# soldasim/BOSS.jl

Measured on AMD Instinct MI355X. Metric: gp_posterior_updates_per_sec (+ acq_evals_per_sec), N=4096 d=8 fp64, higher is better.
Workload: dtype f64; 1 GPU; d=8 synthetic blackbox, GaussianProcess(Matern52) surrogate, N=4096 fp64 posterior update + ExpectedImprovement over 8192 candidates per GPU (BASELINE.json configs[1]+[2]); N=4096, d=8, M_per_gpu=8192, kernel=matern52, parallelism=single GPU: no exchange

## Files before the change

### boss.jl_amd/api.py

```python
from __future__ import annotations

import ctypes as C
import os
from typing import Optional, Sequence

import numpy as np

_HERE = os.path.dirname(os.path.abspath(__file__))
LIB_PATH = os.environ.get("BOSS_LIB_PATH") or os.path.join(_HERE, "libbosship.so")

BOSS_OK, BOSS_E_INVALID, BOSS_E_NO_DEVICE, BOSS_E_NOT_PD, BOSS_E_NEG_VAR, BOSS_E_NOT_FITTED, BOSS_E_ALLOC = range(7)
KERNELS = {"matern32": 0, "matern52": 1, "sqexp": 2}
FIT_NO_SYNC = 1

_c_dp = C.POINTER(C.c_double)
_c_ucp = C.POINTER(C.c_ubyte)

SIGNATURES = {
    "boss_version": (C.c_char_p, []),
    "boss_last_error": (C.c_char_p, []),
    "boss_device_count": (C.c_int, [C.POINTER(C.c_int)]),
    "boss_set_stream": (C.c_int, [C.c_int, C.c_void_p]),
    "boss_device_sync": (C.c_int, [C.c_int]),
    "boss_gp_create": (C.c_int, [C.c_int, C.c_int, C.c_int, C.c_int, _c_dp, _c_dp, _c_ucp, C.POINTER(C.c_void_p)]),
# ... 2216 lines not shown

def _fallbacks(device: int = 0):
    lib = load_library()
    fn = lib.boss_debug_fallbacks
    fn.restype = C.c_int
    fn.argtypes = [C.c_int, C.POINTER(C.c_long), C.POINTER(C.c_int)]
    n, off = C.c_long(0), C.c_int(0)
    _check(fn(device, C.byref(n), C.byref(off)))
    return n.value, off.value


def _set_launches(device: int = 0):
    lib = load_library()
    fn = lib.boss_debug_set_launches
    fn.restype = C.c_int
    fn.argtypes = [C.c_int, C.POINTER(C.c_long), C.POINTER(C.c_long)]
    a, b = C.c_long(0), C.c_long(0)
    fn(device, C.byref(a), C.byref(b))
    return a.value, b.value


def _set_grad_launches(device: int = 0):
    lib = load_library()
    fn = lib.boss_debug_set_grad_launches
    fn.restype = C.c_int
    fn.argtypes = [C.c_int, C.POINTER(C.c_long)]
    a = C.c_long(0)
    fn(device, C.byref(a))
    return a.value


def _acq_path(device: int = 0):
    fn = load_library().boss_debug_acq_path
    fn.restype = C.c_int
    fn.argtypes = [C.c_int, C.POINTER(C.c_int)]
    out = (C.c_int * 5)()
    _check(fn(device, out))
    return tuple(out)


def _acq_prune_set(device: int = 0, min_tiles: int = -1, K: int = -1, s: int = -1, cap: int = -1, slack: Optional[float] = None):
    lib = load_library()
    fn = lib.boss_debug_acq_prune_set
    fn.restype = C.c_int
    fn.argtypes = [C.c_int] * 5
    _check(fn(device, int(min_tiles), int(K), int(s), int(cap)))
    if slack is not None:
        fs = lib.boss_debug_acq_prune_slack
        fs.restype = C.c_int
        fs.argtypes = [C.c_int, C.c_double]
        _check(fs(device, float(slack)))


def _acq_prune_bounds(M: int, device: int = 0):
    fn = load_library().boss_debug_acq_prune_bounds
    fn.restype = C.c_int
    fn.argtypes = [C.c_int, C.c_int, C.c_void_p, C.c_void_p, C.c_void_p]
    mua, vs, ub = np.zeros(M), np.zeros(M), np.zeros(M)
    _check(fn(device, int(M), mua.ctypes.data, vs.ctypes.data, ub.ctypes.data))
    return mua, vs, ub


def _acq_counters(g: GP):
    fn = load_library().boss_debug_acq_counters
    fn.restype = C.c_int
    fn.argtypes = [C.c_void_p, C.POINTER(C.c_long)]
    out = (C.c_long * 4)()
    _check(fn(g._h, out))
    return tuple(out)
```

### boss.jl_amd/csrc/bosship.hip

```cpp
#include "../../include/bosship.h"

#include <hip/hip_runtime.h>

#include <algorithm>
#include <cmath>
#include <cstdint>
#include <cstdio>
#include <cstdlib>
#include <atomic>
#include <chrono>
#include <cstring>
#include <functional>
#include <limits>
#include <map>
#include <mutex>
#include <string>
#include <thread>
#include <vector>

#include "gp_kernels.hpp"
#include "potrf.hpp"
#include "chain.hpp"
#include "small_calls.hpp"
#include "rider.hpp"
// ... 47 lines not shown
        (void)hipDeviceSynchronize();
    }
    return e;
}

constexpr size_t MULTI_RES_OFF = 384;
constexpr size_t FEW_RES_OFF = 400;

struct Workspace {
    void* p = nullptr;
    size_t bytes = 0;
};

struct Ctx {
    int device = -1;
    int logical = -1;
    hipStream_t own_stream = nullptr;
    hipStream_t stream = nullptr;
    hipStream_t side_stream = nullptr;
    std::vector<hipEvent_t> ev_panel, ev_rest;
    hipEvent_t ev_fork = nullptr, ev_up = nullptr;
    unsigned long long* sig_panel = nullptr;
    unsigned long long* sig_panel_host = nullptr;
    unsigned long long sig_seq = 0;
    hipStream_t chain_stream = nullptr, strip_stream = nullptr;
    unsigned long long chain_seq = 0, crit_seq = 0, up_seq = 0;
    int n_cus = 256;
    bool chain_ok = false;
    bool test_drop_chain = false;
    unsigned long long acq_seq = 0;
    unsigned long long few_seq = 0;
    std::mutex slab_mtx;
    void* slab_cache = nullptr;
    size_t slab_cache_bytes = 0;
    void* hostblk_cache = nullptr;
    size_t hostblk_cache_bytes = 0;
    unsigned long long* few_done = nullptr;
    unsigned long long few_done_cnt = 0;
    long set_launches = 0, set_pre_launches = 0;
    long set_grad_launches = 0;
    bool lookahead = true;
    bool prof_on = false;
    std::map<std::string, std::vector<std::pair<hipEvent_t, hipEvent_t>>> prof;
    std::vector<hipEvent_t> ev_pool;
    Workspace vscratch, csc, pred, acq, batchA, batchX, batchMisc, craw, lgA, lgB, lgC, few, setdesc, setmom, gsetdesc, nlatjobs, mceps, meanws, warpws, prunews;
    static constexpr int LLG_BANKS = 4;
    Workspace lgbank[LLG_BANKS - 1][3];
    hipStream_t llg_stream[LLG_BANKS - 1] = {nullptr, nullptr, nullptr};
    hipEvent_t llg_join[LLG_BANKS - 1] = {nullptr, nullptr, nullptr};
    void* pinned = nullptr;
    int prune_last[5] = {0, 0, 0, 0, 0};
    long prune_launches = 0;
    int prune_M = 0;
    struct TrailTab {
        TrailWork* dev = nullptr;
        std::vector<TrailWork> host;
        std::vector<int> off;
    };
    TrailTab trail[65];
    std::mutex mtx;
};

static void chain_quiesce(Ctx* c) {
    if (c->chain_stream) (void)hipStreamSynchronize(c->chain_stream);
    if (c->strip_stream) (void)hipStreamSynchronize(c->strip_stream);
}

static std::mutex g_ctx_mtx;
static std::map<int, Ctx*> g_ctx;

static bool release_cached_slabs() {
    int dev = -1;
    if (hipGetDevice(&dev) != hipSuccess) return false;
    std::vector<void*> blocks;
    {
        std::lock_guard<std::mutex> lk(g_ctx_mtx);
        for (auto& kv : g_ctx) {
            Ctx* c = kv.second;
            if (c->device != dev) continue;
            std::lock_guard<std::mutex> sl(c->slab_mtx);
            if (c->slab_cache) blocks.push_back(c->slab_cache);
            c->slab_cache = nullptr;
            c->slab_cache_bytes = 0;
        }
    }
    for (void* b : blocks) (void)hipFree(b);
    return !blocks.empty();
}
extern "C" int boss_debug_fail_next_alloc(int n) {
    g_fail_allocs.store(n > 0 ? n : 0);
    return BOSS_OK;
}
extern "C" int boss_debug_slab_cache_bytes(int device, size_t* bytes_out) {
    std::lock_guard<std::mutex> lk(g_ctx_mtx);
    auto it = g_ctx.find(device);
    if (bytes_out) *bytes_out = 0;
    if (it != g_ctx.end() && bytes_out) {
        std::lock_guard<std::mutex> sl(it->second->slab_mtx);
        *bytes_out = it->second->slab_cache_bytes;
    }
    return BOSS_OK;
}

extern "C" int boss_debug_set_launches(int device, long* all_out, long* pre_out) {
    std::lock_guard<std::mutex> lk(g_ctx_mtx);
    auto it = g_ctx.find(device);
    if (all_out) *all_out = it != g_ctx.end() ? it->second->set_launches : 0;
    if (pre_out) *pre_out = it != g_ctx.end() ? it->second->set_pre_launches : 0;
    return BOSS_OK;
}

extern "C" int boss_debug_set_grad_launches(int device, long* out) {
    std::lock_guard<std::mutex> lk(g_ctx_mtx);
    auto it = g_ctx.find(device);
    if (out) *out = it != g_ctx.end() ? it->second->set_grad_launches : 0;
    return BOSS_OK;
}

static void ctx_destroy(Ctx* c) {
    if (!c) return;
    if (c->own_stream) (void)hipStreamDestroy(c->own_stream);
    if (c->side_stream) (void)hipStreamDestroy(c->side_stream);
    if (c->chain_stream) (void)hipStreamDestroy(c->chain_stream);
    if (c->strip_stream) (void)hipStreamDestroy(c->strip_stream);
    if (c->ev_fork) (void)hipEventDestroy(c->ev_fork);
    if (c->sig_panel && !c->sig_panel_host) (void)hipFree(c->sig_panel);
    if (c->few_done) (void)hipFree(c->few_done);
    for (auto& t : c->trail)
        if (t.dev) (void)hipFree(t.dev);
    if (c->slab_cache) (void)hipFree(c->slab_cache);
    if (c->hostblk_cache) (void)hipHostFree(c->hostblk_cache);
    if (c->ev_up) (void)hipEventDestroy(c->ev_up);
    for (int i = 0; i < Ctx::LLG_BANKS - 1; ++i) {
        if (c->llg_stream[i]) (void)hipStreamDestroy(c->llg_stream[i]);
        if (c->llg_join[i]) (void)hipEventDestroy(c->llg_join[i]);
    }
    if (c->pinned) (void)hipHostFree(c->pinned);
    delete c;
}

static int ctx_init(Ctx* c) {
    {
        int least = 0, greatest = 0;
        (void)hipDeviceGetStreamPriorityRange(&least, &greatest);
        static const int cu_mask = getenv("BOSS_CU_MASK") ? atoi(getenv("BOSS_CU_MASK")) : 0;
        if (cu_mask) {
            hipDeviceProp_t prop;
            HIPCHK(hipGetDeviceProperties(&prop, c->device));
            const int ncu = prop.multiProcessorCount, words = (ncu + 31) / 32;
            auto make = [&](hipStream_t* st, int lo, int hi) {
                std::vector<uint32_t> m(words, 0u);
                for (int b = lo; b < hi && b < ncu; ++b) m[b / 32] |= 1u << (b % 32);
                return hipExtStreamCreateWithCUMask(st, (uint32_t)words, m.data());
            };
            HIPCHK(make(&c->chain_stream, 0, 16));
            HIPCHK(make(&c->strip_stream, 16, 32));
            HIPCHK(make(&c->own_stream, 32, ncu));
            HIPCHK(make(&c->side_stream, cu_mask >= 2 ? 40 : 32, cu_mask >= 2 ? ncu : ncu - 8));
            c->stream = c->own_stream;
            std::fprintf(stderr, "[bosship] BOSS_CU_MASK=%d: chain on CU bits 0-15, strips on 16-31, main stream on 32-%d, side stream %d-%d\n",
                         cu_mask, ncu - 1, cu_mask >= 2 ? 40 : 32, (cu_mask >= 2 ? ncu : ncu - 8) - 1);
        } else {
        HIPCHK(hipStreamCreateWithPriority(&c->own_stream, hipStreamNonBlocking, greatest));
        c->stream = c->own_stream;
        HIPCHK(hipStreamCreateWithPriority(&c->side_stream, hipStreamNonBlocking, least));
        HIPCHK(hipStreamCreateWithPriority(&c->chain_stream, hipStreamNonBlocking, greatest));
        HIPCHK(hipStreamCreateWithPriority(&c->strip_stream, hipStreamNonBlocking, greatest));
        }
    }
    HIPCHK(hipEventCreateWithFlags(&c->ev_fork, hipEventDisableTiming));
    HIPCHK(hipEventCreateWithFlags(&c->ev_up, hipEventDisableTiming));
    for (int i = 0; i < Ctx::LLG_BANKS - 1; ++i) {
        HIPCHK(hipStreamCreateWithFlags(&c->llg_stream[i], hipStreamNonBlocking));
        HIPCHK(hipEventCreateWithFlags(&c->llg_join[i], hipEventDisableTiming));
    }
    c->lookahead = !(getenv("BOSS_NO_LOOKAHEAD") && atoi(getenv("BOSS_NO_LOOKAHEAD")));
    {
        auto set_nonzero = [](const char* name) {
            const char* v = getenv(name);
            return v && *v && std::strcmp(v, "0") != 0;
        };
        static const bool gate_off = set_nonzero("BOSS_NO_GATE") || set_nonzero("ROCPROF_COUNTER_COLLECTION") || getenv("ROCPROF_COUNTERS") ||
                                     getenv("ROCPROF_COUNTER_GROUPS") || set_nonzero("ROCPROF_ADVANCED_THREAD_TRACE") ||
                                     getenv("ROCPROF_ATT_PARAM_SERIALIZE_ALL") || getenv("ROCP_METRICS") || set_nonzero("AMD_SERIALIZE_KERNEL");
        if (!gate_off) {
            if (set_nonzero("BOSS_DEBUG_WATCH")) {
                unsigned long long* hp = nullptr;
                HIPCHK(hipHostMalloc((void**)&hp, SIG_WORDS * sizeof(unsigned long long), hipHostMallocMapped));
                std::memset(hp, 0, SIG_WORDS * sizeof(unsigned long long));
                HIPCHK(hipHostGetDevicePointer((void**)&c->sig_panel, hp, 0));
                c->sig_panel_host = hp;
#ifdef BOSS_DEBUG_WATCH_BUILD
                HIPCHK(hipMemcpyToSymbol(HIP_SYMBOL(boss::g_dbg), &c->sig_panel, sizeof(void*)));
#endif
                std::thread([hp]() {
                    unsigned long long last[SIG_WORDS] = {0};
                    for (;;) {
                        std::this_thread::sleep_for(std::chrono::milliseconds(500));
                        unsigned long long now[SIG_WORDS];
                        for (int i = 0; i < SIG_WORDS; ++i) now[i] = ((volatile unsigned long long*)hp)[i];
                        if (std::memcmp(now, last, sizeof now) == 0) continue;
                        std::memcpy(last, now, sizeof now);
                        std::fprintf(stderr, "[bosship watch] up %llu wdone %llu panel %llu crit %llu | gate %llu near %llu bulk %llu | strips",
                                     now[SIGW_UP], now[SIGW_WDONE], now[SIGW_PANEL], now[SIGW_CRIT], now[SIGW_GATE], now[SIGW_NEAR], now[SIGW_BULK]);
                        for (int q = 0; q < 8; ++q) std::fprintf(stderr, " %llu", now[SIGW_PROG + SIGW_PROG_STRIDE * q]);
                        std::fprintf(stderr, " | give-ups: first %llu n %llu last %llu; waits ended by mark %llu, by clock %llu", now[SIGW_DBG], now[SIGW_DBG + 1],
                                     now[SIGW_DBG + 2], now[SIGW_DBG + 4], now[SIGW_DBG + 5]);
                        std::fprintf(stderr, "\n");
                    }
                }).detach();
            } else {
                HIPCHK(hipMalloc((void**)&c->sig_panel, SIG_WORDS * sizeof(unsigned long long)));
                HIPCHK(hipMemset(c->sig_panel, 0, SIG_WORDS * sizeof(unsigned long long)));
            }
        }
        c->chain_ok = !gate_off && !set_nonzero("BOSS_NO_CHAIN") && !set_nonzero("HIP_LAUNCH_BLOCKING");
        c->test_drop_chain = set_nonzero("BOSS_TEST_DROP_CHAIN");
        if (c->chain_ok) {
            int* okw = nullptr;
            HIPCHK(hipMalloc((void**)&okw, 4 * sizeof(int)));
            HIPCHK(hipMemset(okw, 0, 4 * sizeof(int)));
            hipStream_t probed[4] = {c->own_stream, c->side_stream, c->chain_stream, c->strip_stream};
            for (int i = 0; i < 4; ++i)
                hipLaunchKernelGGL(chain_probe_wait_kernel, dim3(1), dim3(64), 0, probed[i], c->sig_panel + SIGW_NEAR + 1, 4ull, okw + i);
// ... 469 lines not shown
```

### boss.jl_amd/csrc/host_prune.inc

```

struct PruneCfg {
    int min_tiles = -1;
    int K = 64;
    int s = 1;
    int cap = 1024;
    double slack = 1.0;
};
static PruneCfg g_prune;
constexpr double PRUNE_KMU = 1.2e-4, PRUNE_KVAR = 1e-10;
constexpr size_t PRUNE_RES_OFF = 16;

static bool prune_enabled() {
    static const bool on = !(getenv("BOSS_ACQ_PRUNE") && atoi(getenv("BOSS_ACQ_PRUNE")) == 0);
    static const bool once = [] {
        if (getenv("BOSS_ACQ_PRUNE_BLOCKS")) g_prune.s = std::max(1, atoi(getenv("BOSS_ACQ_PRUNE_BLOCKS")));
        if (getenv("BOSS_ACQ_PRUNE_CAP")) g_prune.cap = std::max(0, atoi(getenv("BOSS_ACQ_PRUNE_CAP")));
        return true;
    }();
    (void)once;
    return on;
}

extern "C" int boss_debug_acq_path(int device, int* out) {
    if (!out) return fail(BOSS_E_INVALID, "out is NULL");
    Ctx* c;
    int rc = get_ctx(device, &c);
    if (rc) return rc;
    std::lock_guard<std::mutex> lk(c->mtx);
    for (int i = 0; i < 5; ++i) out[i] = c->prune_last[i];
    return BOSS_OK;
}
extern "C" int boss_debug_acq_prune_set(int device, int min_tiles, int K, int s, int cap) {
    (void)device;
    (void)prune_enabled();
    const PruneCfg def;
    if (min_tiles != -1) g_prune.min_tiles = min_tiles < -1 ? def.min_tiles : min_tiles;
    if (K != -1) g_prune.K = K < 1 ? def.K : K;
    if (s != -1) g_prune.s = s < 1 ? def.s : s;
    if (cap != -1) g_prune.cap = cap < -1 ? def.cap : cap;
    return BOSS_OK;
}
extern "C" int boss_debug_acq_counters(const boss_gp* g, long* out) {
    if (!g || !out) return fail(BOSS_E_INVALID, "NULL argument");
    out[0] = g->have_winv ? 1 : 0;
    out[1] = g->few_calls;
    out[2] = g_dev_allocs.load();
    out[3] = g->ctx->prune_launches;
    return BOSS_OK;
}
extern "C" int boss_debug_acq_prune_slack(int device, double scale) {
    (void)device;
    if (!(scale >= 0.0)) return fail(BOSS_E_INVALID, "scale must be >= 0");
    g_prune.slack = scale;
    return BOSS_OK;
}
extern "C" int boss_debug_acq_prune_bounds(int device, int M, double* mua_out, double* vars_out, double* ub_out) {
    Ctx* c;
    int rc = get_ctx(device, &c);
    if (rc) return rc;
    std::lock_guard<std::mutex> lk(c->mtx);
    if (M < 1 || M != c->prune_M || !c->prunews.p) return fail(BOSS_E_INVALID, "no pruned attempt with that many candidates");
    HIPCHK(hipStreamSynchronize(c->stream));
    const double* base = (const double*)c->prunews.p;
    if (mua_out) HIPCHK(hipMemcpy(mua_out, base, sizeof(double) * M, hipMemcpyDeviceToHost));
    if (vars_out) HIPCHK(hipMemcpy(vars_out, base + M, sizeof(double) * M, hipMemcpyDeviceToHost));
    if (ub_out) HIPCHK(hipMemcpy(ub_out, base + 2 * (size_t)M, sizeof(double) * M, hipMemcpyDeviceToHost));
    return BOSS_OK;
}

static int prune_few_max_tiles() {
    static const int few_max_tiles = getenv("BOSS_FEW_MAX_TILES") ? atoi(getenv("BOSS_FEW_MAX_TILES")) : 128;
    return few_max_tiles;
}
static bool prune_eligible(const boss_gp* g, const boss_cand* cd, int P, int S, const EiPar& par, bool has_out, bool defer, bool has_mc,
                           const double* dpair) {
    if (!prune_enabled() || has_out || defer || dpair || has_mc || P != 1 || S != 1 || par.mode != 1) return false;
    if (g->aug || g->gibbs || g->ctx->prof_on) return false;
    static const bool no_few = getenv("BOSS_NO_FEW") && atoi(getenv("BOSS_NO_FEW"));
    const int ftiles = (cd->M + 31) / 32, few_max_tiles = prune_few_max_tiles();
    const int min_tiles = g_prune.min_tiles >= 0 ? g_prune.min_tiles : few_max_tiles;
    if (no_few || ftiles <= min_tiles || g->Np < 4 * PRED_RB || g->d > 64 || cd->d != g->d || slab_bn(cd->M, false) != 32) return false;
    if (small_predict_ok(g, cd->M) || cd->M <= g_prune.K || cd->M > PRUNE_THREADS * PRUNE_CPT_MAX) return false;
    if (g_prune.K > 32 * few_max_tiles) return false;
    return g_prune.s < g->Np / PRED_RB;
}

static bool prune_poll(Ctx* c, hipStream_t s, const double* res, unsigned long long want) {
    volatile const unsigned long long* seq = reinterpret_cast<volatile const unsigned long long*>(res) + 4;
    bool got = false;
    for (unsigned long i = 1;; ++i) {
        if (*seq == want) {
            got = true;
            break;
        }
        if ((i & 0x3fff) == 0 && hipStreamQuery(s) != hipErrorNotReady) break;
    }
    std::atomic_thread_fence(std::memory_order_acquire);
    if (!got) {
        (void)hipStreamSynchronize(s);
        got = *seq == want;
    }
    return got;
}

static int prune_avec(boss_gp* g, hipStream_t s, const double** a_out, bool* rebuilt) {
    *rebuilt = false;
    if (g->have_lt && g->avec) {
        *a_out = g->avec;
        return BOSS_OK;
    }
    if (g->prune_a && g->prune_a_np != g->Np) {
        (void)hipStreamSynchronize(s);
        (void)hipFree(g->prune_a);
        g->prune_a = nullptr;
    }
    if (!g->prune_a) {
        if (dev_malloc((void**)&g->prune_a, sizeof(double) * 2 * (size_t)g->Np) != hipSuccess) {
            g->prune_a = nullptr;
            return fail(BOSS_E_ALLOC, "device allocation failed");
        }
        g->prune_a_np = g->Np;
        g->prune_a_gen = ~0ull;
    }
    if (g->prune_a_gen != g->factor_gen) {
        const int nb = g->Np / PRED_RB;
        for (int ib = nb - 1; ib >= 0; --ib)
            hipLaunchKernelGGL(prune_avec_step_kernel, dim3(std::max(1, 2 * ib)), dim3(PRUNE_AVEC_THREADS), 0, s, (const double*)g->A, g->ld, g->Np, g->N,
                               (const double*)g->Dinv2, ib, ib == nb - 1 ? 1 : 0, g->prune_a + g->Np, g->prune_a);
        g->prune_a_gen = g->factor_gen;
        *rebuilt = true;
    }
    *a_out = g->prune_a;
    return BOSS_OK;
}

static int acq_prune_try(boss_gp* g, const boss_cand* cd, const double* mean_dev, const unsigned char* mask_dev, const EiPar& par,
                         bool* done, double* res_out, long* idx_out) {
    *done = false;
    Ctx* c = g->ctx;
    hipStream_t s = c->stream;
    int* last = c->prune_last;
    last[0] = 0;
    last[1] = last[2] = last[4] = 0;
    last[3] = g_prune.s;
    if (g->prune_skip > 0) {
        --g->prune_skip;
        last[0] = 3;
        return BOSS_OK;
    }
    const int M = cd->M, Mp = cd->Mp, d = g->d, Np = g->Np, nch = Np / PRUNE_MU_ROWS, sblk = g_prune.s, K = g_prune.K;
    const int cap = std::min(g_prune.cap, 32 * prune_few_max_tiles()), tiles = (M + 31) / 32;
    const size_t nint = (size_t)round_up(std::max(K, cap), 64);
    const size_t nd = (size_t)4 * M + (size_t)nch * M + 3 * nint + (size_t)d * nint + 2;
    int rc = ws_reserve(c->prunews, sizeof(double) * nd + sizeof(int) * (nint + (size_t)M) + (size_t)M);
    if (rc) return rc;
    rc = ws_reserve(c->csc, sizeof(double) * (size_t)d * Mp);
    if (rc) return rc;
    rc = ws_reserve(c->vscratch, sizeof(double) * (size_t)tiles * 32 * Np);
    if (rc) return rc;
    double* mua = (double*)c->prunews.p;
    double* vars = mua + M;
    double* ub = vars + M;
    unsigned long long* keys = (unsigned long long*)(ub + M);
    double* part = ub + 2 * (size_t)M;
    double* imu = part + (size_t)nch * M;
    double* ivar = imu + nint;
    double* imean = ivar + nint;
    double* icraw = imean + nint;
    double* tpair = icraw + (size_t)d * nint;
    int* sel = (int*)(tpair + 2);
    int* surv = sel + nint;
    unsigned char* insel = (unsigned char*)(surv + M);
    c->prune_M = M;
    double* res = (double*)c->pinned + PRUNE_RES_OFF;

    if (!g->have_dinv) {
        dinv_join(g);
        dinv_launch(g, s);
        g->have_dinv = true;
    }
    dinv_join(g);
    g->dinv_used = true;
    const double* avec = nullptr;
    bool rebuilt = false;
    rc = prune_avec(g, s, &avec, &rebuilt);
    if (rc) return rc;
    last[4] = rebuilt ? 1 : 0;
    c->prune_launches += (rebuilt ? Np / PRED_RB : 0) + 7;
    double* Csc = (double*)c->csc.p;
    hipLaunchKernelGGL(scale_cand_kernel, dim3((Mp + 255) / 256), dim3(256), 0, s, cd->Craw, Csc, g->invlam, g->discrete_dev, d, Mp);
    typedef PredG32 G;
    hipLaunchKernelGGL(prune_head_kernel<G>, dim3(tiles), dim3(G::NTHREADS), PredictLds<G>::BYTES, s, (const double*)g->A, g->ld, Np, g->N,
                       (const double*)g->Dinv2, (const double*)g->Xsc, (const double*)Csc, d, Mp, g->kernel, g->amp2, (double*)c->vscratch.p, M,
                       sblk, vars);
    const size_t mu_lds = sizeof(double) * ((size_t)d + 1) * PRUNE_MU_STAGE;
    auto mu_fn = d <= 16 ? prune_mu_kernel<true> : prune_mu_kernel<false>;
    hipLaunchKernelGGL(mu_fn, dim3((M + PRUNE_MU_CANDS - 1) / PRUNE_MU_CANDS, nch), dim3(256), mu_lds, s, (const double*)g->Xsc, Np, g->N, (const double*)Csc, d, Mp, M,
                       g->kernel, g->amp2, avec, part);
    PrunePar pp;
    pp.coef = par.coefs[0];
    pp.best = par.best;
    pp.amp2 = g->amp2;
    pp.kmu = PRUNE_KMU * g_prune.slack;
    pp.kvar = PRUNE_KVAR * g_prune.slack;
    hipLaunchKernelGGL(prune_bound_kernel, dim3((M + 255) / 256), dim3(256), 0, s, (const double*)part, nch, mean_dev, (const double*)vars, mask_dev, M,
                       pp, mua, ub, keys);
    hipLaunchKernelGGL(prune_select_kernel, dim3(1), dim3(PRUNE_THREADS), 0, s, (const unsigned long long*)keys, M, K, sel, insel);

    boss_cand icd;
    icd.ctx = c;
    icd.d = d;
    auto finish_exact = [&](const int* list, int n) -> int {
        icd.M = n;
        icd.Mp = round_up(n, 64);
        icd.Craw = icraw;
        hipLaunchKernelGGL(prune_gather_kernel, dim3((icd.Mp + 255) / 256), dim3(256), 0, s, list, n, (const double*)cd->Craw, Mp, d, mean_dev,
                           icraw, icd.Mp, mean_dev ? imean : (double*)nullptr);
        return predict_enqueue(g, &icd, mean_dev ? imean : nullptr, imu, ivar, false, nullptr, nullptr, false, true);
    };
    rc = finish_exact(sel, K);
    if (rc) return drain(c, rc);
    unsigned long long seq = ++c->acq_seq;
    hipLaunchKernelGGL(prune_decide_kernel, dim3(1), dim3(PRUNE_THREADS), 0, s, (const int*)sel, K, (const double*)imu, (const double*)ivar,
                       (const double*)mua, mask_dev, par, pp, M, (const double*)ub, (const unsigned char*)insel, surv, tpair, res, seq);
    bool ok = prune_poll(c, s, res, seq);
    hipError_t e = hipGetLastError();
    if (!ok || e != hipSuccess) return fail(BOSS_E_NO_DEVICE, e != hipSuccess ? hipGetErrorString(e) : "the pruned acquisition did not report");
    long cnt = reinterpret_cast<const long*>(res)[2], bad = reinterpret_cast<const long*>(res)[3];
    last[1] = K;
    last[2] = (int)std::min<long>(cnt, 0x7fffffff);
    if (!bad && cnt > 0 && cnt <= cap) {
        rc = finish_exact(surv, (int)cnt);
        if (rc) return drain(c, rc);
        c->prune_launches += 2;
        seq = ++c->acq_seq;
        hipLaunchKernelGGL(prune_merge_kernel, dim3(1), dim3(PRUNE_THREADS), 0, s, (const int*)surv, (int)cnt, (const double*)imu,
                           (const double*)ivar, (const double*)mua, mask_dev, par, pp, (const double*)tpair, res, seq);
        ok = prune_poll(c, s, res, seq);
        e = hipGetLastError();
        if (!ok || e != hipSuccess) return fail(BOSS_E_NO_DEVICE, e != hipSuccess ? hipGetErrorString(e) : "the pruned acquisition did not report");
        bad = reinterpret_cast<const long*>(res)[3];
    }
    if (bad || cnt > cap) {
        g->prune_backoff = g->prune_backoff ? std::min(64, 2 * g->prune_backoff) : 1;
        g->prune_skip = g->prune_backoff;
        last[0] = 2;
        return BOSS_OK;
    }
    g->prune_backoff = 0;
    last[0] = 1;
    *res_out = res[0];
    *idx_out = reinterpret_cast<const long*>(res)[1];
    *done = true;
    return BOSS_OK;
}
```

### boss.jl_amd/csrc/prune_kernels.hpp

```cpp
#pragma once
#include "acq_kernels.hpp"

namespace boss {

template <int NC>
__device__ __forceinline__ void prune_wave_sums(double (&v)[NC], int lane) {
#pragma unroll
    for (int h = NC / 2; h >= 1; h >>= 1) {
        const bool up = (lane & h) != 0;
#pragma unroll
        for (int j = 0; j < h; ++j) {
            const double keep = up ? v[j + h] : v[j], send = up ? v[j] : v[j + h];
            v[j] = keep + __shfl_xor(send, h);
        }
    }
#pragma unroll
    for (int off = NC; off < 64; off <<= 1) v[0] += __shfl_xor(v[0], off);
}
constexpr int PRUNE_AVEC_THREADS = 1024;
__global__ __launch_bounds__(PRUNE_AVEC_THREADS) void prune_avec_step_kernel(const double* __restrict__ A, int ld, int Np, int N,
                                                                             const double* __restrict__ Dinv2, int ib, int first,
                                                                             double* __restrict__ r, double* __restrict__ a) {
    __shared__ double rv[PRED_RB], av[PRED_RB];
    const int tid = threadIdx.x, lane = tid & 63;
// ... 2 lines not shown
    if (tid < PRED_RB) {
        const int i = i0 + tid;
        rv[tid] = first ? (i < N ? A[(size_t)i * ld + Np] : 0.0) : r[i];
    }
    __syncthreads();
    const double* D = Dinv2 + (size_t)ib * PRED_RB * PRED_RB;
    double r4[4];
#pragma unroll
    for (int q = 0; q < 4; ++q) r4[q] = rv[lane + 64 * q];
    {
        double sums[16];
#pragma unroll
        for (int j = 0; j < 16; ++j) {
            const int c = 16 * j + wave;
            const double* col = D + (size_t)c * PRED_RB;
            double sacc = 0.0;
#pragma unroll
            for (int q = 0; q < 4; ++q) {
                if (q >= j / 4) {
                    const int row = lane + 64 * q;
                    const double dv = col[row];
                    sacc = __builtin_fma(row >= c ? dv : 0.0, r4[q], sacc);
                }
            }
            sums[j] = sacc;
        }
        prune_wave_sums<16>(sums, lane);
        if (lane < 16) av[16 * lane + wave] = sums[0];
    }
    __syncthreads();
    if (blockIdx.x == 0 && tid < PRED_RB) a[i0 + tid] = av[tid];
    if (ib == 0) return;
    double a4[4];
#pragma unroll
    for (int q = 0; q < 4; ++q) a4[q] = av[lane + 64 * q];
    double sums[8];
    const int cg0 = blockIdx.x * 128 + wave * 8;
#pragma unroll
    for (int j = 0; j < 8; ++j) {
        const double* col = A + (size_t)(cg0 + j) * ld + i0;
        double sacc = 0.0;
#pragma unroll
        for (int q = 0; q < 4; ++q) sacc = __builtin_fma(col[lane + 64 * q], a4[q], sacc);
        sums[j] = sacc;
    }
    prune_wave_sums<8>(sums, lane);
    if (lane < 8) {
        const int cg = cg0 + lane;
        const double base = first ? (cg < N ? A[(size_t)cg * ld + Np] : 0.0) : r[cg];
        r[cg] = base - sums[0];
    }
}

template <class G>
__global__ __launch_bounds__(G::NTHREADS) __attribute__((amdgpu_waves_per_eu(1, 1))) void prune_head_kernel(
    const double* __restrict__ A, int ld, int Np, int N, const double* __restrict__ Dinv, const double* __restrict__ Xsc,
    const double* __restrict__ Csc, int d, int Mp, int kern, double amp2, double* __restrict__ Vscratch, int M, int sblk,
    double* __restrict__ var_out) {
    static_assert(G::WC == 1 && G::BM == 2 * BLK && G::PM == 2 && G::WR == 4, "written for the 256-row, 32-candidate geometry");
    constexpr int RB = G::BM;
    extern __shared__ double lds[];
    constexpr int BN = G::BN, TM = G::TM, TN = G::TN, LDR = PredictLds<G>::LDR;
    double* Rs = lds;
    double* red = Rs + RB * LDR;
    const int tid = threadIdx.x, lane = tid & 63;
    const int wave = __builtin_amdgcn_readfirstlane(tid >> 6);
    const int wr = wave, wc = 0;
    const int tile = blockIdx.x, c0 = tile * BN;
    double* V = Vscratch + (size_t)tile * sblk * RB * BN;
    double* part = red + 2 * G::WR * G::BN;
#pragma unroll
    for (int u = 0; u < TN * 4; ++u) part[u * G::NTHREADS + tid] = 0.0;
    double* cs = part + (size_t)G::NTHREADS * PredictLds<G>::PART;
    const bool cs_ok = d <= PRED_CS_MAX_D;
    if (cs_ok) {
        for (int idx = tid; idx < d * BN; idx += G::NTHREADS) cs[idx] = Csc[(size_t)(idx / BN) * Mp + c0 + (idx % BN)];
        __syncthreads();
    }
    for (int ib = 0; ib < sblk; ++ib) {
        v4d acc[TM][TN];
#pragma unroll
        for (int m = 0; m < TM; ++m)
#pragma unroll
            for (int n = 0; n < TN; ++n) acc[m][n] = v4d{0.0, 0.0, 0.0, 0.0};
        G::template run<1>(A + (size_t)ib * RB, ld, V, BN, ib * RB, acc);
        double r2[TM][TN][4];
#pragma unroll
        for (int m = 0; m < TM; ++m)
#pragma unroll
            for (int n = 0; n < TN; ++n)
#pragma unroll
                for (int i = 0; i < 4; ++i) r2[m][n][i] = 0.0;
        if (cs_ok) {
            for (int kd0 = 0; kd0 < d; kd0 += 4) {
                double xr[4][TM];
#pragma unroll
                for (int kk = 0; kk < 4; ++kk)
#pragma unroll
                    for (int m = 0; m < TM; ++m)
                        xr[kk][m] = (kd0 + kk < d) ? Xsc[(size_t)(kd0 + kk) * Np + ib * RB + G::row_of(wr, m, lane)] : 0.0;
#pragma unroll
                for (int kk = 0; kk < 4; ++kk) {
                    if (kd0 + kk < d) {
#pragma unroll
                        for (int n = 0; n < TN; ++n)
#pragma unroll
                            for (int i = 0; i < 4; ++i) {
                                const double xc = cs[(kd0 + kk) * BN + G::col_of(wc, n, i, lane)];
#pragma unroll
                                for (int m = 0; m < TM; ++m) {
                                    const double diff = xr[kk][m] - xc;
                                    r2[m][n][i] = __builtin_fma(diff, diff, r2[m][n][i]);
                                }
                            }
                    }
                }
            }
        } else
        for (int kd = 0; kd < d; ++kd) {
            double xr[TM], xc[TN][4];
#pragma unroll
            for (int m = 0; m < TM; ++m) xr[m] = Xsc[(size_t)kd * Np + ib * RB + G::row_of(wr, m, lane)];
#pragma unroll
            for (int n = 0; n < TN; ++n)
#pragma unroll
                for (int i = 0; i < 4; ++i) xc[n][i] = Csc[(size_t)kd * Mp + c0 + G::col_of(wc, n, i, lane)];
#pragma unroll
            for (int m = 0; m < TM; ++m)
#pragma unroll
                for (int n = 0; n < TN; ++n)
#pragma unroll
                    for (int i = 0; i < 4; ++i) {
                        double diff = xr[m] - xc[n][i];
                        r2[m][n][i] = __builtin_fma(diff, diff, r2[m][n][i]);
                    }
        }
#pragma unroll
        for (int m = 0; m < TM; ++m) {
            const int row = G::row_of(wr, m, lane);
            const bool live = (ib * RB + row) < N;
#pragma unroll
            for (int n = 0; n < TN; ++n)
#pragma unroll
                for (int i = 0; i < 4; ++i) {
                    const double ks = live ? amp2 * kappa_r2(kern, r2[m][n][i]) : 0.0;
                    Rs[row * LDR + G::col_of(wc, n, i, lane)] = ks - acc[m][n][i];
                }
        }
        __syncthreads();
        v4d acc2[TM][TN];
#pragma unroll
        for (int m = 0; m < TM; ++m)
#pragma unroll
            for (int n = 0; n < TN; ++n) acc2[m][n] = v4d{0.0, 0.0, 0.0, 0.0};
        G::run_Blds_tri(Dinv + (size_t)ib * RB * RB, RB, Rs, LDR, acc2);
#pragma unroll
        for (int m = 0; m < TM; ++m) {
            const int row = ib * RB + G::tri_row_of(wr, m, lane);
#pragma unroll
            for (int n = 0; n < TN; ++n)
#pragma unroll
                for (int i = 0; i < 4; ++i) {
                    const double v = acc2[m][n][i];
                    if (ib + 1 < sblk) V[(size_t)row * BN + G::col_of(wc, n, i, lane)] = v;
                    double* ps = part + (size_t)(n * 4 + i) * G::NTHREADS + tid;
                    ps[0] = __builtin_fma(v, v, ps[0]);
                }
        }
        __syncthreads();
    }
#pragma unroll
    for (int n = 0; n < TN; ++n)
#pragma unroll
        for (int i = 0; i < 4; ++i) {
            double s = part[(size_t)(n * 4 + i) * G::NTHREADS + tid];
#pragma unroll
            for (int off = 1; off < 16; off <<= 1) s += __shfl_xor(s, off);
            if ((lane & 15) == 0) red[wr * BN + G::col_of(wc, n, i, lane)] = s;
        }
    __syncthreads();
    if (tid < BN) {
        double s = 0.0;
#pragma unroll
        for (int w = 0; w < G::WR; ++w) s += red[w * BN + tid];
        const int j = c0 + tid;
        if (j < M) var_out[j] = amp2 - s + PREDICT_JITTER;
    }
}

constexpr int PRUNE_MU_STAGE = 64, PRUNE_MU_ROWS = 128, PRUNE_MU_CANDS = 512;
template <bool REG>
__global__ __launch_bounds__(256) void prune_mu_kernel(const double* __restrict__ Xsc, int Np, int N, const double* __restrict__ Csc,
                                                       int d, int Mp, int M, int kern, double amp2, const double* __restrict__ a,
                                                       double* __restrict__ part) {
    extern __shared__ double sm[];
    double* xs = sm;
    double* as = sm + (size_t)d * PRUNE_MU_STAGE;
    const int j0 = blockIdx.x * PRUNE_MU_CANDS + threadIdx.x, j1 = j0 + 256;
    const int jc0 = j0 < Mp ? j0 : Mp - 1, jc1 = j1 < Mp ? j1 : Mp - 1;
    const int rbase = blockIdx.y * PRUNE_MU_ROWS;
    double cx0[REG ? 16 : 1], cx1[REG ? 16 : 1];
    if (REG) {
#pragma unroll
        for (int k = 0; k < 16; ++k) {
            cx0[k] = k < d ? Csc[(size_t)k * Mp + jc0] : 0.0;
            cx1[k] = k < d ? Csc[(size_t)k * Mp + jc1] : 0.0;
        }
    }
    double acc0 = 0.0, acc1 = 0.0;
    for (int sub = 0; sub < PRUNE_MU_ROWS / PRUNE_MU_STAGE; ++sub) {
        const int r0 = rbase + sub * PRUNE_MU_STAGE;
        __syncthreads();
        for (int idx = threadIdx.x; idx < d * PRUNE_MU_STAGE; idx += 256)
            xs[idx] = Xsc[(size_t)(idx / PRUNE_MU_STAGE) * Np + r0 + (idx % PRUNE_MU_STAGE)];
        if (threadIdx.x < PRUNE_MU_STAGE) as[threadIdx.x] = (r0 + threadIdx.x < N) ? a[r0 + threadIdx.x] : 0.0;
        __syncthreads();
        if (r0 >= N) continue;
        for (int rg = 0; rg < PRUNE_MU_STAGE; rg += 8) {
            double ra[8], rb[8];
#pragma unroll
            for (int i = 0; i < 8; ++i) ra[i] = rb[i] = 0.0;
            if (REG) {
#pragma unroll
                for (int k = 0; k < 16; ++k)
                    if (k < d) {
#pragma unroll
                        for (int i = 0; i < 8; ++i) {
                            const double x = xs[k * PRUNE_MU_STAGE + rg + i];
                            const double da = x - cx0[k], db = x - cx1[k];
                            ra[i] = __builtin_fma(da, da, ra[i]);
                            rb[i] = __builtin_fma(db, db, rb[i]);
                        }
                    }
            } else {
                for (int k = 0; k < d; ++k) {
                    const double ca = Csc[(size_t)k * Mp + jc0], cb = Csc[(size_t)k * Mp + jc1];
#pragma unroll
                    for (int i = 0; i < 8; ++i) {
                        const double x = xs[k * PRUNE_MU_STAGE + rg + i];
                        const double da = x - ca, db = x - cb;
                        ra[i] = __builtin_fma(da, da, ra[i]);
                        rb[i] = __builtin_fma(db, db, rb[i]);
                    }
                }
            }
#pragma unroll
            for (int i = 0; i < 8; ++i) {
                const double ai = as[rg + i];
                if (r0 + rg + i < N) {
                    acc0 = __builtin_fma(amp2 * kappa_r2(kern, ra[i]), ai, acc0);
                    acc1 = __builtin_fma(amp2 * kappa_r2(kern, rb[i]), ai, acc1);
                }
            }
        }
    }
    if (j0 < M) part[(size_t)blockIdx.y * M + j0] = acc0;
    if (j1 < M) part[(size_t)blockIdx.y * M + j1] = acc1;
}

constexpr int PRUNE_THREADS = 1024;
struct PrunePar {
    double coef, best, amp2;
    double kmu, kvar;
};
__device__ __forceinline__ double prune_dmu(const PrunePar& pp, double muf) {
    return pp.kmu * (fabs(muf) + fabs(pp.best) + fabs(pp.coef) * sqrt(pp.amp2));
}
__device__ __forceinline__ double prune_bound(const PrunePar& pp, double mu, double var) {
    if (var < 0.0) {
        if (var >= -MAX_NEG_VAR) var = 0.0;
        else return NAN;
    }
    const double muf = pp.coef * mu;
    const double vf = pp.coef * pp.coef * (var + pp.kvar * pp.amp2);
    const double sf = sqrt(vf), diff = muf - pp.best + prune_dmu(pp, muf);
    double ei;
    if (diff == 0.0 && sf == 0.0) ei = 0.0;
    else {
        const double z = diff / sf;
        ei = diff * normcdf_dev(z) + sf * normpdf_dev(z);
    }
    return (ei - ei == 0.0) ? ei : NAN;
}
__device__ __forceinline__ unsigned long long prune_key(double v) {
    if (v != v) return ~0ull;
    const unsigned long long b = (unsigned long long)__double_as_longlong(v);
    return (b >> 63) ? ~b : (b | 0x8000000000000000ull);
}
__device__ __forceinline__ int prune_exscan(int v, int* buf, int* total) {
    const int t = threadIdx.x;
    buf[t] = v;
    __syncthreads();
    for (int off = 1; off < PRUNE_THREADS; off <<= 1) {
        const int add = t >= off ? buf[t - off] : 0;
        __syncthreads();
        buf[t] += add;
        __syncthreads();
    }
    const int incl = buf[t];
    *total = buf[PRUNE_THREADS - 1];
    __syncthreads();
    return incl - v;
}

__global__ __launch_bounds__(256) void prune_bound_kernel(const double* __restrict__ part, int nch, const double* __restrict__ mean_s,
                                                          const double* __restrict__ var_s, const unsigned char* __restrict__ mask, int M,
                                                          PrunePar pp, double* __restrict__ mua, double* __restrict__ ub,
                                                          unsigned long long* __restrict__ keys) {
    const int j = blockIdx.x * 256 + threadIdx.x;
    if (j >= M) return;
    double m = mean_s ? mean_s[j] : 0.0;
    for (int ch = 0; ch < nch; ++ch) m += part[(size_t)ch * M + j];
    mua[j] = m;
    const double u = (mask && !mask[j]) ? 0.0 : prune_bound(pp, m, var_s[j]);
    ub[j] = u;
    keys[j] = prune_key(u);
}

__device__ __forceinline__ void prune_hist_add(int* hist, int bin, bool active, int lane) {
    unsigned long long todo = __ballot(active);
    while (todo) {
        const int leader = __ffsll((long long)todo) - 1;
        const int b = __shfl(bin, leader);
        const unsigned long long same = __ballot(active && bin == b);
        if (lane == leader) atomicAdd(&hist[b], (int)__popcll(same));
        todo &= ~same;
    }
}

constexpr int PRUNE_CPT_MAX = 16;
__global__ __launch_bounds__(PRUNE_THREADS) void prune_select_kernel(const unsigned long long* __restrict__ keys, int M, int K,
                                                                     int* __restrict__ sel, unsigned char* __restrict__ insel) {
    __shared__ int hist[256];
    __shared__ int scan[PRUNE_THREADS];
    __shared__ unsigned long long s_prefix;
    __shared__ int s_remaining;
    const int t = threadIdx.x, lane = t & 63;
    unsigned long long kreg[PRUNE_CPT_MAX];
#pragma unroll
    for (int i = 0; i < PRUNE_CPT_MAX; ++i) {
        const int j = t + PRUNE_THREADS * i;
        kreg[i] = j < M ? keys[j] : 0ull;
    }
    if (t == 0) {
        s_prefix = 0ull;
        s_remaining = K;
    }
    __syncthreads();
    for (int pass = 7; pass >= 0; --pass) {
        if (t < 256) hist[t] = 0;
        __syncthreads();
        const unsigned long long prefix = s_prefix;
        const int sh = 8 * pass;
#pragma unroll
        for (int i = 0; i < PRUNE_CPT_MAX; ++i) {
            const unsigned long long k = kreg[i];
            const bool in = (t + PRUNE_THREADS * i < M) && (pass == 7 || (k >> (sh + 8)) == (prefix >> (sh + 8)));
            prune_hist_add(hist, (int)((k >> sh) & 255ull), in, lane);
        }
        __syncthreads();
        const int rem = s_remaining;
        int suf = t < 256 ? hist[t] : 0;
        for (int off = 1; off < 256; off <<= 1) {
            const int add = (t < 256 && t + off < 256) ? hist[t + off] : 0;
            __syncthreads();
            if (t < 256) {
                suf += add;
                hist[t] = suf;
            }
// ... 172 lines not shown
```

Before: 907.0 updates/s.

## Overlap pruned-acquisition mean pass with variance head on side stream using proxy keys

The pruned acquisition path now computes a cheap proxy EI key inside the variance head kernel, using a mean taken from the A matrix's extra column. This lets candidate selection start without waiting for the chunked mean kernel and the bound kernel. The mean and bound kernels move to the side stream and overlap with the head, joining before the decide kernel. This adds event synchronisation and extra LDS accumulators in the head kernel, and it relies on the proxy ordering being a good enough selection key.

```diff
diff --git a/boss.jl_amd/api.py b/boss.jl_amd/api.py
--- a/boss.jl_amd/api.py
+++ b/boss.jl_amd/api.py
@@ -2292,6 +2292,13 @@
         _check(fs(device, float(slack)))
 
 
+def _acq_prune_proxy(mode: int, device: int = 0):
+    fn = load_library().boss_debug_acq_prune_proxy
+    fn.restype = C.c_int
+    fn.argtypes = [C.c_int, C.c_int]
+    _check(fn(device, int(mode)))
+
+
 def _acq_prune_bounds(M: int, device: int = 0):
     fn = load_library().boss_debug_acq_prune_bounds
     fn.restype = C.c_int
diff --git a/boss.jl_amd/csrc/bosship.hip b/boss.jl_amd/csrc/bosship.hip
--- a/boss.jl_amd/csrc/bosship.hip
+++ b/boss.jl_amd/csrc/bosship.hip
@@ -123,6 +123,7 @@
     int prune_last[5] = {0, 0, 0, 0, 0};
     long prune_launches = 0;
     int prune_M = 0;
+    hipEvent_t ev_prune_fork = nullptr, ev_prune_head = nullptr, ev_prune_join = nullptr;
     struct TrailTab {
         TrailWork* dev = nullptr;
         std::vector<TrailWork> host;
@@ -202,6 +203,8 @@
     if (c->slab_cache) (void)hipFree(c->slab_cache);
     if (c->hostblk_cache) (void)hipHostFree(c->hostblk_cache);
     if (c->ev_up) (void)hipEventDestroy(c->ev_up);
+    for (hipEvent_t e : {c->ev_prune_fork, c->ev_prune_head, c->ev_prune_join})
+        if (e) (void)hipEventDestroy(e);
     for (int i = 0; i < Ctx::LLG_BANKS - 1; ++i) {
         if (c->llg_stream[i]) (void)hipStreamDestroy(c->llg_stream[i]);
         if (c->llg_join[i]) (void)hipEventDestroy(c->llg_join[i]);
@@ -241,6 +244,7 @@
     }
     HIPCHK(hipEventCreateWithFlags(&c->ev_fork, hipEventDisableTiming));
     HIPCHK(hipEventCreateWithFlags(&c->ev_up, hipEventDisableTiming));
+    for (hipEvent_t* e : {&c->ev_prune_fork, &c->ev_prune_head, &c->ev_prune_join}) HIPCHK(hipEventCreateWithFlags(e, hipEventDisableTiming));
     for (int i = 0; i < Ctx::LLG_BANKS - 1; ++i) {
         HIPCHK(hipStreamCreateWithFlags(&c->llg_stream[i], hipStreamNonBlocking));
         HIPCHK(hipEventCreateWithFlags(&c->llg_join[i], hipEventDisableTiming));
diff --git a/boss.jl_amd/csrc/host_prune.inc b/boss.jl_amd/csrc/host_prune.inc
--- a/boss.jl_amd/csrc/host_prune.inc
+++ b/boss.jl_amd/csrc/host_prune.inc
@@ -5,6 +5,7 @@
     int s = 1;
     int cap = 1024;
     double slack = 1.0;
+    int proxy = 0;
 };
 static PruneCfg g_prune;
 constexpr double PRUNE_KMU = 1.2e-4, PRUNE_KVAR = 1e-10;
@@ -15,6 +16,7 @@
     static const bool once = [] {
         if (getenv("BOSS_ACQ_PRUNE_BLOCKS")) g_prune.s = std::max(1, atoi(getenv("BOSS_ACQ_PRUNE_BLOCKS")));
         if (getenv("BOSS_ACQ_PRUNE_CAP")) g_prune.cap = std::max(0, atoi(getenv("BOSS_ACQ_PRUNE_CAP")));
+        if (getenv("BOSS_ACQ_PRUNE_PROXY")) g_prune.proxy = std::min(2, std::max(0, atoi(getenv("BOSS_ACQ_PRUNE_PROXY"))));
         return true;
     }();
     (void)once;
@@ -46,6 +48,13 @@
     out[1] = g->few_calls;
     out[2] = g_dev_allocs.load();
     out[3] = g->ctx->prune_launches;
+    return BOSS_OK;
+}
+extern "C" int boss_debug_acq_prune_proxy(int device, int mode) {
+    (void)device;
+    (void)prune_enabled();
+    if (mode < 0 || mode > 2) return fail(BOSS_E_INVALID, "mode must be 0, 1 or 2");
+    g_prune.proxy = mode;
     return BOSS_OK;
 }
 extern "C" int boss_debug_acq_prune_slack(int device, double scale) {
@@ -151,7 +160,7 @@
     const int M = cd->M, Mp = cd->Mp, d = g->d, Np = g->Np, nch = Np / PRUNE_MU_ROWS, sblk = g_prune.s, K = g_prune.K;
     const int cap = std::min(g_prune.cap, 32 * prune_few_max_tiles()), tiles = (M + 31) / 32;
     const size_t nint = (size_t)round_up(std::max(K, cap), 64);
-    const size_t nd = (size_t)4 * M + (size_t)nch * M + 3 * nint + (size_t)d * nint + 2;
+    const size_t nd = (size_t)5 * M + (size_t)nch * M + (size_t)d * Mp + 3 * nint + (size_t)d * nint + 2;
     int rc = ws_reserve(c->prunews, sizeof(double) * nd + sizeof(int) * (nint + (size_t)M) + (size_t)M);
     if (rc) return rc;
     rc = ws_reserve(c->csc, sizeof(double) * (size_t)d * Mp);
@@ -163,7 +172,9 @@
     double* ub = vars + M;
     unsigned long long* keys = (unsigned long long*)(ub + M);
     double* part = ub + 2 * (size_t)M;
-    double* imu = part + (size_t)nch * M;
+    double* mus = part + (size_t)nch * M;
+    double* Csc = mus + M;
+    double* imu = Csc + (size_t)d * Mp;
     double* ivar = imu + nint;
     double* imean = ivar + nint;
     double* icraw = imean + nint;
@@ -179,32 +190,59 @@
         dinv_launch(g, s);
         g->have_dinv = true;
     }
-    dinv_join(g);
     g->dinv_used = true;
-    const double* avec = nullptr;
-    bool rebuilt = false;
-    rc = prune_avec(g, s, &avec, &rebuilt);
-    if (rc) return rc;
-    last[4] = rebuilt ? 1 : 0;
-    c->prune_launches += (rebuilt ? Np / PRED_RB : 0) + 7;
-    double* Csc = (double*)c->csc.p;
-    hipLaunchKernelGGL(scale_cand_kernel, dim3((Mp + 255) / 256), dim3(256), 0, s, cd->Craw, Csc, g->invlam, g->discrete_dev, d, Mp);
-    typedef PredG32 G;
-    hipLaunchKernelGGL(prune_head_kernel<G>, dim3(tiles), dim3(G::NTHREADS), PredictLds<G>::BYTES, s, (const double*)g->A, g->ld, Np, g->N,
-                       (const double*)g->Dinv2, (const double*)g->Xsc, (const double*)Csc, d, Mp, g->kernel, g->amp2, (double*)c->vscratch.p, M,
-                       sblk, vars);
-    const size_t mu_lds = sizeof(double) * ((size_t)d + 1) * PRUNE_MU_STAGE;
-    auto mu_fn = d <= 16 ? prune_mu_kernel<true> : prune_mu_kernel<false>;
-    hipLaunchKernelGGL(mu_fn, dim3((M + PRUNE_MU_CANDS - 1) / PRUNE_MU_CANDS, nch), dim3(256), mu_lds, s, (const double*)g->Xsc, Np, g->N, (const double*)Csc, d, Mp, M,
-                       g->kernel, g->amp2, avec, part);
+    const int proxy = g_prune.proxy;
+    const bool two = proxy != 1 && c->side_stream != nullptr && c->side_stream != s;
+    hipStream_t sb = two ? c->side_stream : s;
+    auto side_drain = [&]() {
+        if (two) (void)hipStreamSynchronize(sb);
+    };
     PrunePar pp;
     pp.coef = par.coefs[0];
     pp.best = par.best;
     pp.amp2 = g->amp2;
     pp.kmu = PRUNE_KMU * g_prune.slack;
     pp.kvar = PRUNE_KVAR * g_prune.slack;
-    hipLaunchKernelGGL(prune_bound_kernel, dim3((M + 255) / 256), dim3(256), 0, s, (const double*)part, nch, mean_dev, (const double*)vars, mask_dev, M,
-                       pp, mua, ub, keys);
+    hipLaunchKernelGGL(scale_cand_kernel, dim3((Mp + 255) / 256), dim3(256), 0, s, cd->Craw, Csc, g->invlam, g->discrete_dev, d, Mp);
+    if (two) {
+        (void)hipEventRecord(c->ev_prune_fork, s);
+        (void)hipStreamWaitEvent(sb, c->ev_prune_fork, 0);
+    }
+    dinv_join(g);
+    const double* avec = nullptr;
+    bool rebuilt = false;
+    typedef PredG32 G;
+    auto head = [&]() {
+        hipLaunchKernelGGL(prune_head_kernel<G>, dim3(tiles), dim3(G::NTHREADS), PredictLds<G>::BYTES, s, (const double*)g->A, g->ld, Np, g->N,
+                           (const double*)g->Dinv2, (const double*)g->Xsc, (const double*)Csc, d, Mp, g->kernel, g->amp2, (double*)c->vscratch.p, M,
+                           sblk, vars, mus, mean_dev, mask_dev, pp, proxy == 2 ? 1 : 0, proxy != 1 ? keys : (unsigned long long*)nullptr);
+        if (two) (void)hipEventRecord(c->ev_prune_head, s);
+    };
+    auto means = [&]() -> int {
+        int r = prune_avec(g, sb, &avec, &rebuilt);
+        if (r) return r;
+        const size_t mu_lds = sizeof(double) * ((size_t)d + 1) * PRUNE_MU_STAGE;
+        auto mu_fn = d <= 16 ? prune_mu_kernel<true> : prune_mu_kernel<false>;
+        hipLaunchKernelGGL(mu_fn, dim3((M + PRUNE_MU_CANDS - 1) / PRUNE_MU_CANDS, nch), dim3(256), mu_lds, sb, (const double*)g->Xsc, Np, g->N,
+                           (const double*)Csc, d, Mp, M, g->kernel, g->amp2, avec, part);
+        return BOSS_OK;
+    };
+    auto bounds = [&]() {
+        if (two) (void)hipStreamWaitEvent(sb, c->ev_prune_head, 0);
+        hipLaunchKernelGGL(prune_bound_kernel, dim3((M + 255) / 256), dim3(256), 0, sb, (const double*)part, nch, mean_dev, (const double*)vars, mask_dev,
+                           M, pp, mua, ub, proxy == 1 ? keys : (unsigned long long*)nullptr);
+        if (two) (void)hipEventRecord(c->ev_prune_join, sb);
+    };
+    if (two) head();
+    rc = means();
+    if (rc) {
+        side_drain();
+        return drain(c, rc);
+    }
+    if (!two) head();
+    bounds();
+    last[4] = rebuilt ? 1 : 0;
+    c->prune_launches += (rebuilt ? Np / PRED_RB : 0) + 7;
     hipLaunchKernelGGL(prune_select_kernel, dim3(1), dim3(PRUNE_THREADS), 0, s, (const unsigned long long*)keys, M, K, sel, insel);
 
     boss_cand icd;
@@ -219,13 +257,20 @@
         return predict_enqueue(g, &icd, mean_dev ? imean : nullptr, imu, ivar, false, nullptr, nullptr, false, true);
     };
     rc = finish_exact(sel, K);
-    if (rc) return drain(c, rc);
+    if (rc) {
+        side_drain();
+        return drain(c, rc);
+    }
+    if (two) (void)hipStreamWaitEvent(s, c->ev_prune_join, 0);
     unsigned long long seq = ++c->acq_seq;
     hipLaunchKernelGGL(prune_decide_kernel, dim3(1), dim3(PRUNE_THREADS), 0, s, (const int*)sel, K, (const double*)imu, (const double*)ivar,
                        (const double*)mua, mask_dev, par, pp, M, (const double*)ub, (const unsigned char*)insel, surv, tpair, res, seq);
     bool ok = prune_poll(c, s, res, seq);
     hipError_t e = hipGetLastError();
-    if (!ok || e != hipSuccess) return fail(BOSS_E_NO_DEVICE, e != hipSuccess ? hipGetErrorString(e) : "the pruned acquisition did not report");
+    if (!ok || e != hipSuccess) {
+        side_drain();
+        return fail(BOSS_E_NO_DEVICE, e != hipSuccess ? hipGetErrorString(e) : "the pruned acquisition did not report");
+    }
     long cnt = reinterpret_cast<const long*>(res)[2], bad = reinterpret_cast<const long*>(res)[3];
     last[1] = K;
     last[2] = (int)std::min<long>(cnt, 0x7fffffff);
diff --git a/boss.jl_amd/csrc/prune_kernels.hpp b/boss.jl_amd/csrc/prune_kernels.hpp
--- a/boss.jl_amd/csrc/prune_kernels.hpp
+++ b/boss.jl_amd/csrc/prune_kernels.hpp
@@ -78,11 +78,40 @@
     }
 }
 
+struct PrunePar {
+    double coef, best, amp2;
+    double kmu, kvar;
+};
+__device__ __forceinline__ unsigned long long prune_key(double v) {
+    if (v != v) return ~0ull;
+    const unsigned long long b = (unsigned long long)__double_as_longlong(v);
+    return (b >> 63) ? ~b : (b | 0x8000000000000000ull);
+}
+__device__ __forceinline__ unsigned long long prune_proxy_key(const PrunePar& pp, double mu, double var, bool masked, bool reversed) {
+    if (masked) return 0ull;
+    if (var < 0.0) {
+        if (var >= -MAX_NEG_VAR) var = 0.0;
+        else return ~0ull;
+    }
+    const double sf = sqrt(pp.coef * pp.coef * var), diff = pp.coef * mu - pp.best;
+    double ei = 0.0, z = 0.0;
+    if (!(diff == 0.0 && sf == 0.0)) {
+        z = diff / sf;
+        ei = diff * normcdf_dev(z) + sf * normpdf_dev(z);
+    }
+    if (!(ei - ei == 0.0)) return ~0ull;
+    unsigned long long k = ei > 0.0 ? prune_key(ei) : prune_key(z < 0.0 ? z : -0.0);
+    if (k == 0ull) k = 1ull;
+    if (k == ~0ull) k = ~1ull;
+    return reversed ? ~k : k;
+}
+
 template <class G>
 __global__ __launch_bounds__(G::NTHREADS) __attribute__((amdgpu_waves_per_eu(1, 1))) void prune_head_kernel(
     const double* __restrict__ A, int ld, int Np, int N, const double* __restrict__ Dinv, const double* __restrict__ Xsc,
     const double* __restrict__ Csc, int d, int Mp, int kern, double amp2, double* __restrict__ Vscratch, int M, int sblk,
-    double* __restrict__ var_out) {
+    double* __restrict__ var_out, double* __restrict__ mus_out, const double* __restrict__ mean_s,
+    const unsigned char* __restrict__ mask, PrunePar pp, int reversed, unsigned long long* __restrict__ keys) {
     static_assert(G::WC == 1 && G::BM == 2 * BLK && G::PM == 2 && G::WR == 4, "written for the 256-row, 32-candidate geometry");
     constexpr int RB = G::BM;
     extern __shared__ double lds[];
@@ -96,7 +125,7 @@
     double* V = Vscratch + (size_t)tile * sblk * RB * BN;
     double* part = red + 2 * G::WR * G::BN;
 #pragma unroll
-    for (int u = 0; u < TN * 4; ++u) part[u * G::NTHREADS + tid] = 0.0;
+    for (int u = 0; u < 2 * TN * 4; ++u) part[u * G::NTHREADS + tid] = 0.0;
     double* cs = part + (size_t)G::NTHREADS * PredictLds<G>::PART;
     const bool cs_ok = d <= PRED_CS_MAX_D;
     if (cs_ok) {
@@ -183,6 +212,7 @@
 #pragma unroll
         for (int m = 0; m < TM; ++m) {
             const int row = ib * RB + G::tri_row_of(wr, m, lane);
+            const double zr = A[(size_t)row * ld + Np];
 #pragma unroll
             for (int n = 0; n < TN; ++n)
 #pragma unroll
@@ -191,6 +221,8 @@
                     if (ib + 1 < sblk) V[(size_t)row * BN + G::col_of(wc, n, i, lane)] = v;
                     double* ps = part + (size_t)(n * 4 + i) * G::NTHREADS + tid;
                     ps[0] = __builtin_fma(v, v, ps[0]);
+                    double* pz = ps + (size_t)TN * 4 * G::NTHREADS;
+                    pz[0] = __builtin_fma(v, zr, pz[0]);
                 }
         }
         __syncthreads();
@@ -199,18 +231,32 @@
     for (int n = 0; n < TN; ++n)
 #pragma unroll
         for (int i = 0; i < 4; ++i) {
-            double s = part[(size_t)(n * 4 + i) * G::NTHREADS + tid];
-#pragma unroll
-            for (int off = 1; off < 16; off <<= 1) s += __shfl_xor(s, off);
-            if ((lane & 15) == 0) red[wr * BN + G::col_of(wc, n, i, lane)] = s;
+            double s = part[(size_t)(n * 4 + i) * G::NTHREADS + tid], z = part[(size_t)(TN * 4 + n * 4 + i) * G::NTHREADS + tid];
+#pragma unroll
+            for (int off = 1; off < 16; off <<= 1) {
+                s += __shfl_xor(s, off);
+                z += __shfl_xor(z, off);
+            }
+            if ((lane & 15) == 0) {
+                red[wr * BN + G::col_of(wc, n, i, lane)] = s;
+                red[G::WR * BN + wr * BN + G::col_of(wc, n, i, lane)] = z;
+            }
         }
     __syncthreads();
     if (tid < BN) {
-        double s = 0.0;
-#pragma unroll
-        for (int w = 0; w < G::WR; ++w) s += red[w * BN + tid];
+        double s = 0.0, z = 0.0;
+#pragma unroll
+        for (int w = 0; w < G::WR; ++w) {
+            s += red[w * BN + tid];
+            z += red[G::WR * BN + w * BN + tid];
+        }
         const int j = c0 + tid;
-        if (j < M) var_out[j] = amp2 - s + PREDICT_JITTER;
+        if (j < M) {
+            const double var = amp2 - s + PREDICT_JITTER;
+            var_out[j] = var;
+            mus_out[j] = z;
+            if (keys) keys[j] = prune_proxy_key(pp, (mean_s ? mean_s[j] : 0.0) + z, var, mask && !mask[j], reversed != 0);
+        }
     }
 }
 
@@ -285,10 +331,6 @@
 }
 
 constexpr int PRUNE_THREADS = 1024;
-struct PrunePar {
-    double coef, best, amp2;
-    double kmu, kvar;
-};
 __device__ __forceinline__ double prune_dmu(const PrunePar& pp, double muf) {
     return pp.kmu * (fabs(muf) + fabs(pp.best) + fabs(pp.coef) * sqrt(pp.amp2));
 }
@@ -307,11 +349,6 @@
         ei = diff * normcdf_dev(z) + sf * normpdf_dev(z);
     }
     return (ei - ei == 0.0) ? ei : NAN;
-}
-__device__ __forceinline__ unsigned long long prune_key(double v) {
-    if (v != v) return ~0ull;
-    const unsigned long long b = (unsigned long long)__double_as_longlong(v);
-    return (b >> 63) ? ~b : (b | 0x8000000000000000ull);
 }
 __device__ __forceinline__ int prune_exscan(int v, int* buf, int* total) {
     const int t = threadIdx.x;
@@ -340,7 +377,7 @@
     mua[j] = m;
     const double u = (mask && !mask[j]) ? 0.0 : prune_bound(pp, m, var_s[j]);
     ub[j] = u;
-    keys[j] = prune_key(u);
+    if (keys) keys[j] = prune_key(u);
 }
 
 __device__ __forceinline__ void prune_hist_add(int* hist, int bin, bool active, int lane) {
```

Result: no change. 910.9 updates/s (median of 3 runs) (+0.4%).
